# pbs-plus/pbs-plus

Hardware: AMD Instinct MI355X
Metric: GiB/s ingested through CDC+SHA-256 (higher is better)
Workload: dtype u32

## Files before the change

### pbs_plus_amd/csrc/kernels.hip

```cpp
#include "kernel_util.h"
#include "kernels.h"
#include "ring_queue.h"

namespace pbsk {

__device__ __forceinline__ uint32_t rotr(uint32_t x, int n) { return __builtin_rotateright32(x, n); }

__device__ __forceinline__ uint32_t xor3(uint32_t a, uint32_t b, uint32_t c) {
    return __builtin_amdgcn_bitop3_b32(a, b, c, 0x96);
}
__device__ __forceinline__ uint32_t maj3(uint32_t a, uint32_t b, uint32_t c) {
    return __builtin_amdgcn_bitop3_b32(a, b, c, 0xE8);
}
__device__ __forceinline__ uint32_t ch3(uint32_t e, uint32_t f, uint32_t g) { return g ^ (e & (f ^ g)); }

__device__ constexpr uint32_t kSha256K[64] = {
    0x428a2f98, 0x71374491, 0xb5c0fbcf, 0xe9b5dba5, 0x3956c25b, 0x59f111f1, 0x923f82a4, 0xab1c5ed5,
    0xd807aa98, 0x12835b01, 0x243185be, 0x550c7dc3, 0x72be5d74, 0x80deb1fe, 0x9bdc06a7, 0xc19bf174,
    0xe49b69c1, 0xefbe4786, 0x0fc19dc6, 0x240ca1cc, 0x2de92c6f, 0x4a7484aa, 0x5cb0a9dc, 0x76f988da,
    0x983e5152, 0xa831c66d, 0xb00327c8, 0xbf597fc7, 0xc6e00bf3, 0xd5a79147, 0x06ca6351, 0x14292967,
    0x27b70a85, 0x2e1b2138, 0x4d2c6dfc, 0x53380d13, 0x650a7354, 0x766a0abb, 0x81c2c92e, 0x92722c85,
    0xa2bfe8a1, 0xa81a664b, 0xc24b8b70, 0xc76c51a3, 0xd192e819, 0xd6990624, 0xf40e3585, 0x106aa070,
    0x19a4c116, 0x1e376c08, 0x2748774c, 0x34b0bcb5, 0x391c0cb3, 0x4ed8aa4a, 0x5b9cca4f, 0x682e6ff3,
    0x748f82ee, 0x78a5636f, 0x84c87814, 0x8cc70208, 0x90befffa, 0xa4506ceb, 0xbef9a3f7, 0xc67178f2};

__device__ __forceinline__ uint32_t sha256_sched(uint32_t (&W)[16], int i) {
    const uint32_t w15 = W[(i + 1) & 15], w2 = W[(i + 14) & 15];
    const uint32_t s0 = xor3(rotr(w15, 7), rotr(w15, 18), w15 >> 3);
    const uint32_t s1 = xor3(rotr(w2, 17), rotr(w2, 19), w2 >> 10);
    const uint32_t w = W[i & 15] + s0 + W[(i + 9) & 15] + s1;
    W[i & 15] = w;
    return w;
}

#define SHA256_ROUND(a, b, c, d, e, f, g, h, wk)                                   \
    do {                                                                           \
        const uint32_t t1_ = (h) + xor3(rotr(e, 6), rotr(e, 11), rotr(e, 25)) + ch3(e, f, g) + (wk); \
        const uint32_t t2_ = xor3(rotr(a, 2), rotr(a, 13), rotr(a, 22)) + maj3(a, b, c); \
        (d) += t1_;                                                                \
        (h) = t1_ + t2_;                                                           \
    } while (0)

__device__ __forceinline__ void sha256_compress(uint32_t (&H)[8], uint32_t (&W)[16]) {
    uint32_t a = H[0], b = H[1], c = H[2], d = H[3], e = H[4], f = H[5], g = H[6], h = H[7];
#pragma unroll
    for (int i = 0; i < 64; i += 8) {
        uint32_t wk[8];
#pragma unroll
        for (int j = 0; j < 8; ++j) wk[j] = ((i + j < 16) ? W[i + j] : sha256_sched(W, i + j)) + kSha256K[i + j];
        SHA256_ROUND(a, b, c, d, e, f, g, h, wk[0]);
        SHA256_ROUND(h, a, b, c, d, e, f, g, wk[1]);
        SHA256_ROUND(g, h, a, b, c, d, e, f, wk[2]);
        SHA256_ROUND(f, g, h, a, b, c, d, e, wk[3]);
        SHA256_ROUND(e, f, g, h, a, b, c, d, wk[4]);
        SHA256_ROUND(d, e, f, g, h, a, b, c, wk[5]);
        SHA256_ROUND(c, d, e, f, g, h, a, b, wk[6]);
        SHA256_ROUND(b, c, d, e, f, g, h, a, wk[7]);
    }
    H[0] += a; H[1] += b; H[2] += c; H[3] += d; H[4] += e; H[5] += f; H[6] += g; H[7] += h;
}

__device__ __forceinline__ void sha256_iv(uint32_t (&H)[8]) {
    H[0] = 0x6a09e667; H[1] = 0xbb67ae85; H[2] = 0x3c6ef372; H[3] = 0xa54ff53a;
    H[4] = 0x510e527f; H[5] = 0x9b05688c; H[6] = 0x1f83d9ab; H[7] = 0x5be0cd19;
}

__device__ uint32_t kIdleBlock[32];

__device__ __forceinline__ void sha256_request_block(const uint8_t *p, uint32_t (&R)[17], uint32_t &sel) {
    const uint32_t o = (uint32_t)((uintptr_t)p & 3u);
    const gvec4_ptr q = (gvec4_ptr)(p - o);
    const u32x4_a4 v0 = q[0], v1 = q[1], v2 = q[2], v3 = q[3];
    R[0] = v0.x; R[1] = v0.y; R[2] = v0.z; R[3] = v0.w;
    R[4] = v1.x; R[5] = v1.y; R[6] = v1.z; R[7] = v1.w;
    R[8] = v2.x; R[9] = v2.y; R[10] = v2.z; R[11] = v2.w;
    R[12] = v3.x; R[13] = v3.y; R[14] = v3.z; R[15] = v3.w;
    R[16] = ((gword_ptr)(p - o))[o ? 16 : 15];
    sel = ((o) << 24) | ((o + 1) << 16) | ((o + 2) << 8) | (o + 3);
}

__device__ __forceinline__ void sha256_tail_words(const uint8_t *base, uint64_t len, uint64_t off, bool last, uint32_t (&R)[17]) {
    const int64_t rem = (int64_t)len - (int64_t)off;
    const uint32_t valid = rem <= 0 ? 0u : (rem >= 64 ? 64u : (uint32_t)rem);
    uint32_t q[17];
#pragma unroll
    for (int j = 0; j < 17; ++j) q[j] = 0;
    uint32_t o = 0;
    if (valid) {
        const uint8_t *p = base + off;
        o = (uint32_t)((uintptr_t)p & 3u);
        const gword_ptr a = (gword_ptr)(p - o);
        const uint32_t jmax = (o + valid - 1u) >> 2;
#pragma unroll
        for (int j = 0; j < 17; ++j) q[j] = a[min((uint32_t)j, jmax)];
    }
    const uint32_t sh = o * 8u;
#pragma unroll
    for (int j = 0; j < 16; ++j) {
        uint32_t w = sh ? ((q[j] >> sh) | (q[j + 1] << (32u - sh))) : q[j];
        const int32_t k = (int32_t)valid - 4 * j;
        const uint32_t mask = k >= 4 ? 0xffffffffu : (k <= 0 ? 0u : ((1u << (8 * k)) - 1u));
        w &= mask;
        if (rem >= 0 && rem < 64 && k >= 0 && k < 4) w |= 0x80u << (8 * k);
        R[j] = w;
    }
    if (last) {
        const uint64_t bits = len * 8;
        R[14] = __builtin_bswap32((uint32_t)(bits >> 32));
        R[15] = __builtin_bswap32((uint32_t)bits);
    }
    R[16] = 0;
}

struct RecordSource {
    static constexpr bool kRing = false;
    pbsgpu_record *recs;
    const uint4 *qdesc;
    __device__ __forceinline__ void get(uint32_t i, const uint8_t *&ptr, uint64_t &len, uint8_t *&dst) const {
        const uint4 d = qdesc[i];
        ptr = reinterpret_cast<const uint8_t *>(((uint64_t)d.y << 32) | d.x);
        len = d.z;
        dst = recs[d.w].digest;
    }
};
struct SegmentSource {
    static constexpr bool kRing = false;
    const uint8_t *data;
    const pbsgpu_segment *segs;
    uint8_t *digests;
    __device__ __forceinline__ void get(uint32_t i, const uint8_t *&ptr, uint64_t &len, uint8_t *&dst) const {
        ptr = data + segs[i].offset;
        len = segs[i].length;
        dst = digests + (uint64_t)i * 32;
    }
};


struct RingProbe {
    uint32_t n = 0, idle = 0, act = 0;
    unsigned long long c0 = 0, w0 = 0;
};
__device__ __forceinline__ void ring_probe_step(const RingSource &src, RingProbe &pb, const bool busy, const int slot, const int lane,
                                                const uint32_t active = 0) {
    pb.idle |= busy ? 0u : 1u;
    pb.act += active;
    if (++pb.n < kRingProbeSteps) return;
    const unsigned long long c = clock64(), w = wall_clock64();
    if (!pb.idle && pb.w0 != 0ull && lane == 0 && src.probe) {
        atomicAdd(src.probe + slot, (unsigned long long)kRingProbeSteps);
        atomicAdd(src.probe + slot + 1, c - pb.c0);
        atomicAdd(src.probe + slot + 2, w - pb.w0);
        if (slot == 0) atomicAdd(src.probe + 8, (unsigned long long)pb.act);
    }
    pb.n = 0;
    pb.act = 0;
    pb.idle = 0;
    pb.c0 = c;
    pb.w0 = w;
}

template <typename Source>
__global__ __launch_bounds__(64) void k_sha256(Source src, const uint32_t *nitems_p, uint32_t nitems_imm,
                                               uint32_t *queue, const uint32_t *wg_limit, uint32_t whole_chip) {
    if (wg_limit) {
        const uint32_t lim = *wg_limit;
        if (whole_chip ? lim == 0 : blockIdx.x >= lim * 2u) return;
    }
    const int lane = threadIdx.x & 63;
    const uint32_t nitems = nitems_p ? *nitems_p : nitems_imm;

    const uint8_t *base = nullptr;
    uint64_t len = 0;
    uint64_t blk = 0, nblk = 0;
    uint8_t *dst = nullptr;
    bool have = false;
    bool exhausted = false;

    uint32_t R[17];
    uint32_t sel = 0x00010203u;
#pragma unroll
    for (int j = 0; j < 17; ++j) R[j] = 0;

    uint32_t H[8];
    sha256_iv(H);

    auto load_block = [&]() {
        const uint64_t off = blk * 64;
        if (off + 64 <= len) {
            const uint8_t *p = base + off;
            const uint32_t o = (uint32_t)((uintptr_t)p & 3u);
            const gvec4_ptr q = (gvec4_ptr)(p - o);
            const u32x4_a4 v0 = q[0], v1 = q[1], v2 = q[2], v3 = q[3];
            R[0] = v0.x; R[1] = v0.y; R[2] = v0.z; R[3] = v0.w;
            R[4] = v1.x; R[5] = v1.y; R[6] = v1.z; R[7] = v1.w;
            R[8] = v2.x; R[9] = v2.y; R[10] = v2.z; R[11] = v2.w;
            R[12] = v3.x; R[13] = v3.y; R[14] = v3.z; R[15] = v3.w;
            R[16] = o ? ((gword_ptr)(p - o))[16] : 0u;
            sel = ((o) << 24) | ((o + 1) << 16) | ((o + 2) << 8) | (o + 3);
        } else {
            sha256_tail_words(base, len, off, blk + 1 == nblk, R);
            sel = 0x00010203u;
        }
    };

    auto acquire = [&](bool need) {
        const unsigned long long m = __ballot(need);
        if (m == 0) return;
        const uint32_t first = wave_claim(queue, m, (uint32_t)__popcll(m), lane);
        if (need) {
            const uint32_t i = first + wave_rank(m, lane);
            if (i < nitems) {
                src.get(i, base, len, dst);
                blk = 0;
                nblk = (len + 8) / 64 + 1;
                have = true;
            } else {
                exhausted = true;
                have = false;
            }
        }
    };

    acquire(true);
    if (have) load_block();

    while (__any(have)) {
        uint32_t W[16];
#pragma unroll
        for (int j = 0; j < 16; ++j) W[j] = __builtin_amdgcn_perm(R[j + 1], R[j], sel);
        const bool cur = have;
        const bool cur_last = have && (blk + 1 == nblk);
        uint8_t *cur_dst = dst;

        if (have) {
            if (!cur_last) ++blk; else have = false;
        }
        acquire(!have && !exhausted);
        if (have) load_block();

        if (cur) sha256_compress(H, W);

        if (cur_last) {
            uint32_t *o = reinterpret_cast<uint32_t *>(cur_dst);
#pragma unroll
            for (int j = 0; j < 8; ++j) o[j] = __builtin_bswap32(H[j]);
            sha256_iv(H);
        }
    }
}

__global__ __launch_bounds__(512) void k_sha256_lanes(RingSource src) {
    const int lane = threadIdx.x & 63;
    const uint8_t *base = nullptr, *base2 = nullptr;
    uint64_t len = 0, blk = 0, nblk = 0;
    uint32_t len1 = 0, pages = 0xffffffffu, poll_ctr = 0;
    uint8_t *dst = nullptr;
    bool have = false, exhausted = false;
    uint32_t R[17];
    uint32_t sel = 0x00010203u;
#pragma unroll
    for (int j = 0; j < 17; ++j) R[j] = 0;
    uint32_t H[8];
    sha256_iv(H);

    auto load_block = [&]() {
        const uint64_t off = blk * 64;
        const uint8_t *bb = (off < len1) ? base : base2;
        if (off + 64 <= len) {
            sha256_request_block(bb + off, R, sel);
        } else {
            sha256_tail_words(bb, len, off, blk + 1 == nblk, R);
            sel = 0x00010203u;
        }
    };
    auto acquire = [&](bool need) {
        if (__ballot(need) == 0) return;
        if (__ballot(have) != 0 && ((++poll_ctr) & src.poll_mask) != 0u) return;
        uint32_t sh;
        const int32_t avail = ring_queue_avail(&src.ctl->sq, sh);
        const unsigned long long mn = __ballot(need);
        if (avail > 0) {
            const uint32_t cnt = min((uint32_t)__popcll(mn), (uint32_t)avail);
            const uint32_t first = ring_cas_claim(&src.ctl->shead, sh, cnt, mn, lane);
            if (first != 0xffffffffu) {
                const uint32_t rank = wave_rank(mn, lane);
                const bool got = need && rank < cnt;
                uint4 e0, e1;
                ring_desc_load(src.sdesc, (first + rank) & src.smask, got, e0, e1);
                ring_desc_take(src, got, e0, e1, base, base2, len, len1, dst, pages);
                blk = got ? 0ull : blk;
                nblk = got ? ((uint64_t)e0.z + 8u) / 64u + 1u : nblk;
                have = have | got;
            }
        } else if (ring_stop_raised(src) && ring_drained_after_stop(&src.ctl->sq)) {
            exhausted = exhausted | need;
        }
    };

    const bool probe_on = src.probe != nullptr && blockIdx.x == 0 && threadIdx.x < 64;
    uint32_t pn = 0, pidle = 0, pact = 0;
    unsigned long long pw0 = 0;
    acquire(true);
    if (have) load_block();
    for (;;) {
        if (probe_on) {
            const unsigned long long hm = __ballot(have);
            pidle |= hm ? 0u : 1u;
            pact += (uint32_t)__popcll(hm);
            if (++pn >= kRingProbeSteps) {
                const unsigned long long w = wall_clock64();
                if (!pidle && pw0 != 0ull && lane == 0) {
                    atomicAdd(src.probe + 6, (unsigned long long)kRingProbeSteps);
                    atomicAdd(src.probe + 7, w - pw0);
                    atomicAdd(src.probe + 9, (unsigned long long)pact);
                }
                pn = 0; pidle = 0; pact = 0; pw0 = w;
            }
        }
        if (!__any(have)) {
            if (__ballot(!exhausted) == 0ull) break;
            __builtin_amdgcn_s_sleep(48);
            poll_ctr = 0;
            acquire(!exhausted);
            if (have) load_block();
            continue;
        }
        uint32_t W[16];
#pragma unroll
        for (int j = 0; j < 16; ++j) W[j] = __builtin_amdgcn_perm(R[j + 1], R[j], sel);
        const bool cur = have;
        const bool cur_last = have && (blk + 1 == nblk);
        uint8_t *cur_dst = dst;
        if (have) {
            if (!cur_last) ++blk; else have = false;
        }
        if (cur_last) ring_release_pages(src, pages);
        acquire(!have && !exhausted);
        if (have) load_block();
        if (cur) sha256_compress(H, W);
        if (cur_last) {
            PBSK_GLOBAL uint32_t *o = (PBSK_GLOBAL uint32_t *)cur_dst;
#pragma unroll
            for (int j = 0; j < 8; ++j) o[j] = __builtin_bswap32(H[j]);
            ring_cell_publish(o);
            sha256_iv(H);
        }
    }
}

template <typename Source, bool DENSE>
__global__ __launch_bounds__(DENSE ? 512 : 256) void k_sha256_pair(Source src, const uint32_t *nitems_p, uint32_t nitems_imm,
                                                                   uint32_t *queue, const uint32_t *wg_limit) {
    if (wg_limit) {
        const uint32_t lim = *wg_limit;
        if (DENSE ? lim == 0 : blockIdx.x >= lim) return;
    }
    constexpr int NP = DENSE ? 4 : 2;
    __shared__ uint4 wkbuf_[NP][2][16][64];
    __shared__ uint32_t ctrl_[NP][2][64];
    __shared__ uint8_t *dstp_[NP][2][64];
    __shared__ uint32_t alive[NP][2];
    __shared__ uint32_t curw[NP][2];
    const int lane = threadIdx.x & 63;
    const int wave = threadIdx.x >> 6;
    const int pr = (wave & 1) | (wave >= 4 ? 2 : 0);
    const bool producer = (wave >= 2 && wave < 6);
    auto &wkbuf = wkbuf_[pr];
    auto &ctrl = ctrl_[pr];
    auto &dstp = dstp_[pr];
    auto any_alive = [&](const int pb) -> uint32_t {
        uint32_t a = alive[0][pb] | alive[1][pb];
        if constexpr (DENSE) a |= alive[2][pb] | alive[3][pb];
        return a;
    };

    if (producer) {
        const uint32_t nitems = nitems_p ? *nitems_p : nitems_imm;
        const uint8_t *base = nullptr;
        uint64_t len = 0, blk = 0, nblk = 0;
        uint8_t *dst = nullptr;
        bool have = false, exhausted = false;
        [[maybe_unused]] const uint8_t *base2 = nullptr;
        [[maybe_unused]] uint32_t len1 = 0, pages = 0xffffffffu, claim = 0;
        [[maybe_unused]] uint32_t claimed = 0;
        [[maybe_unused]] unsigned long long idle_since = 0;
        [[maybe_unused]] uint32_t hb_seen = 0;
        constexpr int D = 2;
        uint32_t R[D][17];
        uint32_t selv[D], cflag[D];
        uint8_t *dstv[D];
        [[maybe_unused]] uint32_t pagesv[D];
#pragma unroll
        for (int s = 0; s < D; ++s) {
#pragma unroll
            for (int j = 0; j < 17; ++j) R[s][j] = 0;
            selv[s] = 0x00010203u;
            cflag[s] = 0;
            dstv[s] = nullptr;
            pagesv[s] = 0xffffffffu;
        }

        constexpr uint32_t kReserve = 16;
        uint32_t res_next = 0, res_end = 0;
        [[maybe_unused]] uint32_t poll_ctr = 0;
        auto acquire = [&](bool need) {
            if constexpr (Source::kRing) {
                if (__ballot(need) == 0) return;
                if (__ballot(have) != 0 && ((++poll_ctr) & src.poll_mask) != 0u) return;
                const bool long_only = src.long_bytes != 0u && src.xp == 0u && (lane & 15) == 0;
                const bool elig = need && claimed == 0u;
                if (src.long_bytes && __ballot(elig)) {
                    uint32_t lh;
                    int32_t avail = ring_queue_avail(&src.ctl->lq, lh) - (int32_t)src.long_spill;
                    if (avail > 0 && src.xp != 0u && (uint32_t)avail <= src.xp_pairs &&
                        __hip_atomic_load(&src.ctl->xp_busy, __ATOMIC_RELAXED, __HIP_MEMORY_SCOPE_AGENT) < src.xp_pairs)
                        avail = 0;
                    if (avail > 0) {
                        const unsigned long long mn = __ballot(elig);
                        const uint32_t cnt = min((uint32_t)__popcll(mn), (uint32_t)avail);
                        const uint32_t first = ring_cas_claim(&src.ctl->lhead, lh, cnt, mn, lane);
                        if (first != 0xffffffffu) {
                            const uint32_t rank = wave_rank(mn, lane);
                            const bool tk = elig && rank < cnt;
                            uint4 e0, e1;
                            ring_desc_load(src.ldesc, (first + rank) & src.lmask, tk, e0, e1);
                            ring_desc_take(src, tk, e0, e1, base, base2, len, len1, dst, pages);
                            blk = tk ? 0ull : blk;
                            nblk = tk ? ((uint64_t)e0.z + 8u) / 64u + 1u : nblk;
                            have = have | tk;
                            need = need && !tk;
                        }
                    }
                }
                const bool want = need && !claimed && !long_only;
                const unsigned long long mw = __ballot(want);
                if (mw) {
                    uint32_t first = 0;
                    const int leader = __ffsll((long long)mw) - 1;
                    if (lane == leader) {
                        const uint32_t cnt = (uint32_t)__popcll(mw);
                        first = atomicAdd(&src.ctl->head, cnt);
                        if (((first + cnt) ^ first) >> 8)
                            __hip_atomic_store(const_cast<uint32_t *>(src.heartbeat) + 32, first + cnt, __ATOMIC_RELAXED,
                                               __HIP_MEMORY_SCOPE_SYSTEM);
                    }
                    first = __shfl(first, leader, 64);
                    if (want) {
                        claim = first + wave_rank(mw, lane);
                        claimed = 1u;
                    }
                }
                if (__ballot(need) == 0) return;
                const unsigned long long ts = __hip_atomic_load(&src.ctl->tail_stop,
                                                                __ATOMIC_RELAXED, __HIP_MEMORY_SCOPE_AGENT);
                const uint32_t tail = (uint32_t)ts, stop = (uint32_t)(ts >> 32);
                const bool ready = need && claimed != 0u && (int32_t)(tail - claim) > 0;
                if (__ballot(ready)) __atomic_thread_fence(__ATOMIC_ACQUIRE);
                uint4 d0, d1;
                ring_desc_load(src.desc, claim & src.qmask, ready, d0, d1);
                const bool got = ready && d0.z != 0u;
                claimed = ready ? 0u : claimed;
                ring_desc_take(src, got, d0, d1, base, base2, len, len1, dst, pages);
                blk = got ? 0ull : blk;
                nblk = got ? ((uint64_t)d0.z + 8u) / 64u + 1u : nblk;
                have = have | got;
                bool leave = need && !ready && stop != 0u;
                if (src.long_bytes && src.xp == 0u && __ballot(leave) && !ring_drained_after_stop(&src.ctl->lq)) leave = false;
                exhausted = exhausted | leave;
                return;
            }
            const unsigned long long m = __ballot(need);
            if (m == 0) return;
            uint32_t first = 0;
            uint32_t avail = 0;
            if constexpr (DENSE) {
                const uint32_t cnt = (uint32_t)__popcll(m);
                avail = res_end - res_next;
                if (cnt > avail) first = wave_claim(queue, m, cnt - avail + kReserve, lane);
            } else {
                first = wave_claim(queue, m, (uint32_t)__popcll(m), lane);
            }
            if (need) {
                uint32_t i = first + wave_rank(m, lane);
                if constexpr (DENSE) {
                    const uint32_t r = wave_rank(m, lane);
                    i = r < avail ? res_next + r : first + (r - avail);
                }
                if (i < nitems) {
                    if constexpr (!Source::kRing) src.get(i, base, len, dst);
                    blk = 0;
                    nblk = (len + 8) / 64 + 1;
                    have = true;
                } else {
                    exhausted = true;
                    have = false;
                }
            }
            if constexpr (DENSE) {
                const uint32_t cnt = (uint32_t)__popcll(m);
                if (cnt > avail) {
                    res_next = first + (cnt - avail);
                    res_end = res_next + kReserve;
                } else {
                    res_next += cnt;
                }
            }
        };
        auto prep = [&](const int s) {
            acquire(!have && !exhausted);
            uint32_t c = 0;
            const uint8_t *p = reinterpret_cast<const uint8_t *>(kIdleBlock);
            const uint8_t *bb = base;
            uint64_t off = 0;
            bool tail = false, last = false;
            if (have) {
                off = blk * 64;
                if constexpr (Source::kRing) bb = (off < len1) ? base : base2;
                last = blk + 1 == nblk;
                if (off + 64 <= len) p = bb + off;
                else tail = true;
                c = 1u | (last ? 2u : 0u);
                dstv[s] = dst;
                if constexpr (Source::kRing) pagesv[s] = pages;
                if (++blk == nblk) have = false;
            }
            sha256_request_block(p, R[s], selv[s]);
            if (tail) {
                sha256_tail_words(bb, len, off, last, R[s]);
                selv[s] = 0x00010203u;
            }
            cflag[s] = c;
        };

#pragma unroll
        for (int s = 0; s < D; ++s) prep(s);
        bool drained = false;
        [[maybe_unused]] bool wg_busy = false;
        [[maybe_unused]] RingProbe probe;
        [[maybe_unused]] const bool probe_on = blockIdx.x == 0 && wave == 2;
        while (!drained) {
#pragma unroll
            for (int s = 0; s < D; ++s) {
                {
                    constexpr int kBufMask = 1;
                    const int pb = s & kBufMask;
                    uint32_t W[16];
#pragma unroll
                    for (int j = 0; j < 16; ++j) {
                        W[j] = __builtin_amdgcn_perm(R[s][j + 1], R[s][j], selv[s]);
                        asm volatile("" : "+v"(W[j]));
                    }
                    __builtin_amdgcn_sched_barrier(0);
                    const uint32_t c = cflag[s];
                    uint8_t *cur_dst = dstv[s];
                    if constexpr (Source::kRing) {
                        if (c & 2u) ring_release_pages(src, pagesv[s]);
                    }
                    prep(s);
                    const bool any_cur = __any(c & 1u);
                    if (any_cur) {
#pragma unroll
                        for (int q = 0; q < 16; ++q) {
                            uint32_t x[4];
#pragma unroll
                            for (int j = 0; j < 4; ++j) {
                                const int t = 4 * q + j;
                                x[j] = ((t < 16) ? W[t] : sha256_sched(W, t)) + kSha256K[t];
                            }
                            wkbuf[pb][q][lane] = make_uint4(x[0], x[1], x[2], x[3]);
                        }
                    }
                    ctrl[pb][lane] = c;
                    dstp[pb][lane] = cur_dst;
                    bool live = any_cur;
                    if constexpr (Source::kRing) {
                        const bool wave_done = __ballot(!exhausted) == 0ull;
                        live = any_cur || !wave_done;
                        if (!any_cur && !wave_done) {
                            const unsigned long long now = wall_clock64();
                            if (idle_since == 0) idle_since = now;
                            if (blockIdx.x == 0 && wave == 2 && now - idle_since > src.idle_ticks) {
                                uint32_t *hbw = const_cast<uint32_t *>(src.heartbeat);
                                const uint32_t hb = __hip_atomic_load(hbw + kHbBeat, __ATOMIC_RELAXED, __HIP_MEMORY_SCOPE_SYSTEM);
                                if (hb != hb_seen) {
                                    hb_seen = hb;
                                    idle_since = now;
                                } else {
                                    if (lane == 0) __hip_atomic_store(hbw + kHbIntent, 1u, __ATOMIC_RELAXED, __HIP_MEMORY_SCOPE_SYSTEM);
                                    __atomic_thread_fence(__ATOMIC_SEQ_CST);
                                    __threadfence_system();
                                    const uint32_t hb2 = __hip_atomic_load(hbw + kHbBeat, __ATOMIC_RELAXED, __HIP_MEMORY_SCOPE_SYSTEM);
                                    const uint32_t enq = __hip_atomic_load(hbw + kHbRoundsEnq, __ATOMIC_RELAXED, __HIP_MEMORY_SCOPE_SYSTEM);
                                    const uint32_t done = __hip_atomic_load(&src.ctl->rounds_done, __ATOMIC_RELAXED, __HIP_MEMORY_SCOPE_AGENT);
                                    if (hb2 != hb || enq != done) {
                                        if (lane == 0) __hip_atomic_store(hbw + kHbIntent, 0u, __ATOMIC_RELAXED, __HIP_MEMORY_SCOPE_SYSTEM);
                                        hb_seen = hb2;
                                        idle_since = now;
                                    } else if (lane == 0) {
                                        __hip_atomic_store(&src.ctl->stop, 2u, __ATOMIC_RELEASE, __HIP_MEMORY_SCOPE_AGENT);
                                        __hip_atomic_store(hbw + kHbCommitted, 1u, __ATOMIC_RELAXED, __HIP_MEMORY_SCOPE_SYSTEM);
                                    }
                                }
                            }
                            if (!wg_busy) __builtin_amdgcn_s_sleep(48);
                        } else {
                            idle_since = 0;
                        }
                        if (lane == 0) curw[pr][pb] = any_cur ? 1u : 0u;
                        if (probe_on) ring_probe_step(src, probe, any_cur, 0, lane, (uint32_t)__popcll(__ballot(c & 1u)));
                    }
                    if (lane == 0) alive[pr][pb] = live ? 1u : 0u;
                    __syncthreads();
                    drained = drained || __builtin_amdgcn_readfirstlane(any_alive(pb)) == 0u;
                    if constexpr (Source::kRing) {
                        uint32_t w = curw[0][pb] | curw[1][pb];
                        if constexpr (DENSE) w |= curw[2][pb] | curw[3][pb];
                        wg_busy = w != 0u;
                    }
                }
            }
        }
    } else {
        uint32_t H[8];
        sha256_iv(H);
        struct Blk {
            uint32_t al, c;
            uint8_t *d;
            uint4 wk[16];
        };
        auto fetch = [&](Blk &x, const int pb) {
            x.al = any_alive(pb);
            x.c = ctrl[pb][lane];
            x.d = dstp[pb][lane];
#pragma unroll
            for (int q = 0; q < 16; ++q) x.wk[q] = wkbuf[pb][q][lane];
        };
        auto rounds = [&](const Blk &x) {
            if (x.c & 1u) {
                uint32_t a = H[0], b = H[1], cc = H[2], dd = H[3], e = H[4], f = H[5], g = H[6], h = H[7];
#pragma unroll
                for (int q = 0; q < 16; q += 2) {
                    SHA256_ROUND(a, b, cc, dd, e, f, g, h, x.wk[q].x);
                    SHA256_ROUND(h, a, b, cc, dd, e, f, g, x.wk[q].y);
                    SHA256_ROUND(g, h, a, b, cc, dd, e, f, x.wk[q].z);
                    SHA256_ROUND(f, g, h, a, b, cc, dd, e, x.wk[q].w);
                    SHA256_ROUND(e, f, g, h, a, b, cc, dd, x.wk[q + 1].x);
                    SHA256_ROUND(dd, e, f, g, h, a, b, cc, x.wk[q + 1].y);
                    SHA256_ROUND(cc, dd, e, f, g, h, a, b, x.wk[q + 1].z);
                    SHA256_ROUND(b, cc, dd, e, f, g, h, a, x.wk[q + 1].w);
                }
                H[0] += a; H[1] += b; H[2] += cc; H[3] += dd; H[4] += e; H[5] += f; H[6] += g; H[7] += h;
                if (x.c & 2u) {
                    PBSK_GLOBAL uint32_t *o = (PBSK_GLOBAL uint32_t *)x.d;
#pragma unroll
                    for (int j = 0; j < 8; ++j) o[j] = __builtin_bswap32(H[j]);
                    if constexpr (Source::kRing) ring_cell_publish(o);
                    sha256_iv(H);
                }
            }
        };
        Blk A, B;
        __syncthreads();
        fetch(A, 0);
        for (;;) {
            if (!A.al) break;
            __syncthreads();
            fetch(B, 1);
            __builtin_amdgcn_sched_barrier(0);
            rounds(A);
            if (!B.al) break;
            __syncthreads();
            fetch(A, 0);
            __builtin_amdgcn_sched_barrier(0);
            rounds(B);
        }
    }
}

#define XP_R(n, x0, x1, x2, x3, kw)                                                     \
    "v_xad_u32 %[nz], " x3 ", %[role], " kw "\n\t"                                      \
    "v_alignbit_b32 %[r1], " x0 ", " x0 ", %[sh1]\n\t"                                  \
    "v_alignbit_b32 %[r2], " x0 ", " x0 ", %[sh2]\n\t"                                  \
    "v_add_u32_dpp %[p], " x1 ", %[nz] quad_perm:[1,0,3,2] row_mask:0xf bank_mask:0xf\n\t" \
    "v_alignbit_b32 %[r3], " x0 ", " x0 ", %[sh3]\n\t"                                  \
    "v_bitop3_b32 %[sel], " x0 ", " x2 ", %[role] bitop3:0x78\n\t"                      \
    "v_bitop3_b32 %[sg], %[r1], %[r2], %[r3] bitop3:0x96\n\t"                           \
    "v_bitop3_b32 %[f], %[sel], " x1 ", " x2 " bitop3:0xca\n\t"                         \
    "v_add3_u32 " n ", %[sg], %[f], %[p]\n\t"
#define XP_TEMPS                                                                                                   \
    [nz] "=&v"(nz), [r1] "=&v"(r1), [r2] "=&v"(r2), [r3] "=&v"(r3), [p] "=&v"(p), [sel] "=&v"(sel), [sg] "=&v"(sg), \
        [f] "=&v"(f)
struct XpRole {
    uint32_t sh1, sh2, sh3, role;
};
template <bool START>
__device__ __forceinline__ void xp_round4(uint32_t &x0, uint32_t &x1, uint32_t &x2, uint32_t &x3, const uint4 kw, const XpRole &R,
                                          const uint32_t hb1 = 0, const uint32_t hb0 = 0) {
    uint32_t n0, n1, n2, n3, nz, r1, r2, r3, p, sel, sg, f;
    if constexpr (START) {
        asm(XP_R("%[n0]", "%[x0]", "%[x1]", "%[x2]", "%[x3]", "%[k0]")
            "v_bitop3_b32 %[n0], %[role], %[hb1], %[n0] bitop3:0xca\n\t"
            XP_R("%[n1]", "%[n0]", "%[x0]", "%[x1]", "%[x2]", "%[k1]")
            "v_bitop3_b32 %[n1], %[role], %[hb0], %[n1] bitop3:0xca\n\t"
            XP_R("%[n2]", "%[n1]", "%[n0]", "%[x0]", "%[x1]", "%[k2]")
            XP_R("%[n3]", "%[n2]", "%[n1]", "%[n0]", "%[x0]", "%[k3]")
            : [n0] "=&v"(n0), [n1] "=&v"(n1), [n2] "=&v"(n2), [n3] "=&v"(n3), XP_TEMPS
            : [x0] "v"(x0), [x1] "v"(x1), [x2] "v"(x2), [x3] "v"(x3), [k0] "v"(kw.x), [k1] "v"(kw.y), [k2] "v"(kw.z), [k3] "v"(kw.w),
              [sh1] "v"(R.sh1), [sh2] "v"(R.sh2), [sh3] "v"(R.sh3), [role] "v"(R.role), [hb1] "v"(hb1), [hb0] "v"(hb0));
    } else {
        asm(XP_R("%[n0]", "%[x0]", "%[x1]", "%[x2]", "%[x3]", "%[k0]")
            XP_R("%[n1]", "%[n0]", "%[x0]", "%[x1]", "%[x2]", "%[k1]")
            XP_R("%[n2]", "%[n1]", "%[n0]", "%[x0]", "%[x1]", "%[k2]")
            XP_R("%[n3]", "%[n2]", "%[n1]", "%[n0]", "%[x0]", "%[k3]")
            : [n0] "=&v"(n0), [n1] "=&v"(n1), [n2] "=&v"(n2), [n3] "=&v"(n3), XP_TEMPS
            : [x0] "v"(x0), [x1] "v"(x1), [x2] "v"(x2), [x3] "v"(x3), [k0] "v"(kw.x), [k1] "v"(kw.y), [k2] "v"(kw.z), [k3] "v"(kw.w),
              [sh1] "v"(R.sh1), [sh2] "v"(R.sh2), [sh3] "v"(R.sh3), [role] "v"(R.role));
    }
    x0 = n3; x1 = n2; x2 = n1; x3 = n0;
}
__device__ __forceinline__ void xp_round2(uint32_t &x0, uint32_t &x1, uint32_t &x2, uint32_t &x3, const uint32_t kw, const XpRole &R) {
    uint32_t n0, n1, nz, r1, r2, r3, p, sel, sg, f;
    asm(XP_R("%[n0]", "%[x0]", "%[x1]", "%[x2]", "%[x3]", "%[k0]")
        XP_R("%[n1]", "%[n0]", "%[x0]", "%[x1]", "%[x2]", "%[k0]")
        : [n0] "=&v"(n0), [n1] "=&v"(n1), XP_TEMPS
        : [x0] "v"(x0), [x1] "v"(x1), [x2] "v"(x2), [x3] "v"(x3), [k0] "v"(kw), [sh1] "v"(R.sh1), [sh2] "v"(R.sh2), [sh3] "v"(R.sh3),
          [role] "v"(R.role));
    x3 = x1; x2 = x0; x1 = n0; x0 = n1;
}
__device__ __forceinline__ uint32_t xp_sel(uint32_t role, uint32_t a, uint32_t b) { return __builtin_amdgcn_bitop3_b32(role, b, a, 0xCA); }

template <typename Source>
__global__ __launch_bounds__(256) void k_sha256_xpair(Source src, const uint32_t *nitems_p, uint32_t nitems_imm, uint32_t *queue,
                                                      const uint32_t *wg_limit) {
    if (wg_limit && *wg_limit == 0) return;
    __shared__ uint4 wkbuf_[2][2][2][16][64];
    __shared__ uint32_t ctrl_[2][2][2][32];
    __shared__ uint8_t *dstp_[2][2][2][32];
    __shared__ uint32_t alive[2][2];
    __shared__ uint32_t curw[2][2];
    const int lane = threadIdx.x & 63;
    const int wave = threadIdx.x >> 6;
    const int pr = wave & 1;
    const bool producer = wave >= 2;
    const bool roleB = (lane & 1) != 0;
    const int ci = lane >> 1;
    auto &wkbuf = wkbuf_[pr];
    auto &ctrl = ctrl_[pr];
    auto &dstp = dstp_[pr];
    auto any_alive = [&](const int pb) -> uint32_t { return alive[0][pb] | alive[1][pb]; };
    for (int i = threadIdx.x; i < 2 * 2 * 2 * 16 * 32; i += 256) {
        const int row = 2 * (i & 31) + 1, q = (i >> 5) & 15, pl = (i >> 9) & 1, pb = (i >> 10) & 1, pp = (i >> 11) & 1;
        wkbuf_[pp][pb][pl][q][row] = make_uint4(1u, 1u, 1u, 1u);
    }
    __syncthreads();

    if (producer) {
        const uint32_t nitems = nitems_p ? *nitems_p : nitems_imm;
        const uint8_t *base = nullptr;
        uint64_t len = 0, blk = 0, nblk = 0;
        uint8_t *dst = nullptr;
        bool have = false, exhausted = false;
        [[maybe_unused]] const uint8_t *base2 = nullptr;
        [[maybe_unused]] uint32_t len1 = 0, pages = 0xffffffffu;
        [[maybe_unused]] unsigned long long idle_since = 0;
        [[maybe_unused]] uint32_t poll_ctr = 0;
        constexpr int D = 2;
        uint32_t R[D][17];
        uint32_t selv[D], cflag[D];
        uint8_t *dstv[D];
        [[maybe_unused]] uint32_t pagesv[D];
#pragma unroll
        for (int s = 0; s < D; ++s) {
#pragma unroll
            for (int j = 0; j < 17; ++j) R[s][j] = 0;
            selv[s] = 0x00010203u;
            cflag[s] = 0;
            dstv[s] = nullptr;
            pagesv[s] = 0xffffffffu;
        }
        auto acquire = [&](bool need) {
            if (__ballot(need) == 0) return;
            bool got = false;
            if constexpr (Source::kRing) {
                if (__ballot(have) != 0 && ((++poll_ctr) & src.poll_mask) != 0u) return;
                uint32_t lh;
                const int32_t avail = ring_queue_avail(&src.ctl->lq, lh);
                const unsigned long long mn = __ballot(need);
                if (avail > 0) {
                    const uint32_t cnt = min((uint32_t)__popcll(mn), (uint32_t)avail);
                    const uint32_t first = ring_cas_claim(&src.ctl->lhead, lh, cnt, mn, lane);
                    if (first != 0xffffffffu) {
                        const uint32_t rank = wave_rank(mn, lane);
                        got = need && rank < cnt;
                        uint4 e0, e1;
                        ring_desc_load(src.ldesc, (first + rank) & src.lmask, got, e0, e1);
                        ring_desc_take(src, got, e0, e1, base, base2, len, len1, dst, pages);
                        if (lane == __ffsll((long long)mn) - 1) atomicAdd(&src.ctl->xp_busy, cnt);
                    }
                } else if (ring_stop_raised(src) && ring_drained_after_stop(&src.ctl->lq)) {
                    exhausted = exhausted | need;
                }
            } else {
                const unsigned long long m = __ballot(need);
                const uint32_t first = wave_claim(queue, m, (uint32_t)__popcll(m), lane);
                if (need) {
                    const uint32_t i = first + wave_rank(m, lane);
                    if (i < nitems) {
                        src.get(i, base, len, dst);
                        got = true;
                    } else {
                        exhausted = true;
                    }
                }
            }
            const int srcl = lane & ~1;
            const bool pgot = __shfl((int)got, srcl, 64) != 0;
            exhausted = __shfl((int)exhausted, srcl, 64) != 0;
            if (__ballot(pgot)) {
                const uint64_t b1 = (uint64_t)__shfl((unsigned long long)reinterpret_cast<uintptr_t>(base), srcl, 64);
                const uint64_t ln = (uint64_t)__shfl((unsigned long long)len, srcl, 64);
                const uint64_t ds = (uint64_t)__shfl((unsigned long long)reinterpret_cast<uintptr_t>(dst), srcl, 64);
                if (pgot) {
                    base = reinterpret_cast<const uint8_t *>(b1);
                    len = ln;
                    dst = reinterpret_cast<uint8_t *>(ds);
                }
                if constexpr (Source::kRing) {
                    const uint64_t b2 = (uint64_t)__shfl((unsigned long long)reinterpret_cast<uintptr_t>(base2), srcl, 64);
                    const uint32_t l1 = (uint32_t)__shfl((int)len1, srcl, 64);
                    const uint32_t pg = (uint32_t)__shfl((int)pages, srcl, 64);
                    if (pgot) {
                        base2 = reinterpret_cast<const uint8_t *>(b2);
                        len1 = l1;
                        pages = pg;
                    }
                }
                if (pgot) {
                    nblk = (len + 8) / 64 + 1;
                    blk = roleB ? 1ull : 0ull;
                    have = blk < nblk;
                }
            }
        };
        auto prep = [&](const int s) {
            const unsigned long long hm = __ballot(have);
            const bool pair_busy = ((hm >> (lane & ~1)) & 3ull) != 0ull;
            acquire(!roleB && !pair_busy && !exhausted);
            uint32_t c = 0;
            const uint8_t *p = reinterpret_cast<const uint8_t *>(kIdleBlock);
            const uint8_t *bb = base;
            uint64_t off = 0;
            bool tail = false, last = false;
            if (have) {
                off = blk * 64;
                if constexpr (Source::kRing) bb = (off < len1) ? base : base2;
                last = blk + 1 == nblk;
                if (off + 64 <= len) p = bb + off;
                else tail = true;
                c = 1u | (last ? 2u : 0u);
                dstv[s] = dst;
                if constexpr (Source::kRing) pagesv[s] = pages;
                blk += 2;
                if (blk >= nblk) have = false;
            }
            sha256_request_block(p, R[s], selv[s]);
            if (tail) {
                sha256_tail_words(bb, len, off, last, R[s]);
                selv[s] = 0x00010203u;
            }
            cflag[s] = c;
        };
        const int wrow = lane & ~1, wplane = lane & 1;

#pragma unroll
        for (int s = 0; s < D; ++s) prep(s);
        bool drained = false;
        [[maybe_unused]] bool wg_busy = false;
        [[maybe_unused]] RingProbe probe;
        [[maybe_unused]] const bool probe_on = blockIdx.x == 0 && wave == 2;
        while (!drained) {
#pragma unroll
            for (int s = 0; s < D; ++s) {
                {
                    const int pb = s & 1;
                    uint32_t W[16];
#pragma unroll
                    for (int j = 0; j < 16; ++j) {
                        W[j] = __builtin_amdgcn_perm(R[s][j + 1], R[s][j], selv[s]);
                        asm volatile("" : "+v"(W[j]));
                    }
                    __builtin_amdgcn_sched_barrier(0);
                    const uint32_t c = cflag[s];
                    uint8_t *cur_dst = dstv[s];
                    if constexpr (Source::kRing) {
                        {
                            const unsigned long long mdone = __ballot((c & 2u) != 0u);
                            if (mdone && lane == (__ffsll((long long)mdone) - 1)) atomicSub(&src.ctl->xp_busy, (uint32_t)__popcll(mdone));
                        }
                        if (c & 2u) ring_release_pages(src, pagesv[s]);
                    }
                    prep(s);
                    const bool any_cur = __any(c & 1u);
                    if (any_cur) {
#pragma unroll
                        for (int q = 0; q < 16; ++q) {
                            uint32_t x[4];
#pragma unroll
                            for (int j = 0; j < 4; ++j) {
                                const int t = 4 * q + j;
                                x[j] = ((t < 16) ? W[t] : sha256_sched(W, t)) + kSha256K[t];
                            }
                            wkbuf[pb][wplane][q][wrow] = make_uint4(x[0], x[1], x[2], x[3]);
                        }
                    }
                    ctrl[pb][wplane][ci] = c;
                    dstp[pb][wplane][ci] = cur_dst;
                    bool live = any_cur;
                    if constexpr (Source::kRing) {
                        const bool wave_done = __ballot(!exhausted) == 0ull;
                        live = any_cur || !wave_done;
                        if (!any_cur && !wave_done && !wg_busy) __builtin_amdgcn_s_sleep(48);
                        if (lane == 0) curw[pr][pb] = any_cur ? 1u : 0u;
                        if (probe_on) ring_probe_step(src, probe, any_cur, 3, lane);
                    }
                    if (lane == 0) alive[pr][pb] = live ? 1u : 0u;
                    __syncthreads();
                    drained = drained || __builtin_amdgcn_readfirstlane(any_alive(pb)) == 0u;
                    if constexpr (Source::kRing) wg_busy = (curw[0][pb] | curw[1][pb]) != 0u;
                }
            }
        }
    } else {
        const XpRole R{roleB ? 2u : 6u, roleB ? 13u : 11u, roleB ? 22u : 25u, roleB ? 0xffffffffu : 0u};
        const uint32_t role = R.role;
        uint32_t ivr[4];
        ivr[0] = roleB ? 0x6a09e667u : 0x510e527fu;
        ivr[1] = roleB ? 0xbb67ae85u : 0x9b05688cu;
        ivr[2] = roleB ? 0x3c6ef372u : 0x1f83d9abu;
        ivr[3] = roleB ? 0xa54ff53au : 0x5be0cd19u;
        uint32_t HR[4] = {ivr[0], ivr[1], ivr[2], ivr[3]};
        struct Blk {
            uint32_t al, c;
            uint8_t *d;
            uint4 wk[16];
        };
        auto fetch = [&](Blk &x, const int pb, const int plane) {
            x.al = any_alive(pb);
            x.c = ctrl[pb][plane][ci];
            x.d = dstp[pb][plane][ci];
#pragma unroll
            for (int q = 0; q < 16; ++q) x.wk[q] = wkbuf[pb][plane][q][lane];
        };
        auto rounds = [&](const Blk &x) {
            if (x.c & 1u) {
                uint32_t x0 = xp_sel(role, HR[0], HR[2]), x1 = xp_sel(role, HR[1], HR[3]), x2 = HR[2], x3 = HR[3];
                xp_round4<true>(x0, x1, x2, x3, x.wk[0], R, HR[1], HR[0]);
#pragma unroll
                for (int g = 1; g < 16; ++g) xp_round4<false>(x0, x1, x2, x3, x.wk[g], R);
                const uint32_t o63 = x0, o62 = x1, o61 = x2, o60 = x3;
                xp_round2(x0, x1, x2, x3, x.wk[15].w, R);
                HR[0] += xp_sel(role, o63, x0);
                HR[1] += xp_sel(role, o62, x1);
                HR[2] += xp_sel(role, o61, o63);
                HR[3] += xp_sel(role, o60, o62);
                if (x.c & 2u) {
                    PBSK_GLOBAL uint32_t *o = (PBSK_GLOBAL uint32_t *)x.d + (roleB ? 0 : 4);
#pragma unroll
                    for (int j = 0; j < 4; ++j) o[j] = __builtin_bswap32(HR[j]);
                    if constexpr (Source::kRing) ring_cell_publish((PBSK_GLOBAL uint32_t *)x.d);
#pragma unroll
                    for (int j = 0; j < 4; ++j) HR[j] = ivr[j];
                }
            }
        };
        Blk E0, O0, E1, O1;
        __syncthreads();
        fetch(E0, 0, 0);
        for (;;) {
            if (!E0.al) break;
            fetch(O0, 0, 1);
            __builtin_amdgcn_sched_barrier(0);
            rounds(E0);
            __syncthreads();
            fetch(E1, 1, 0);
            __builtin_amdgcn_sched_barrier(0);
            rounds(O0);
            if (!E1.al) break;
            fetch(O1, 1, 1);
            __builtin_amdgcn_sched_barrier(0);
            rounds(E1);
            __syncthreads();
            fetch(E0, 0, 0);
            __builtin_amdgcn_sched_barrier(0);
            rounds(O1);
        }
    }
}

__global__ __launch_bounds__(1024) void k_order(const uint8_t *data, const pbsgpu_segment *segs, const pbsgpu_record *recs,
                                                const uint32_t *nrec_p, uint32_t shift, uint4 *qdesc, uint32_t *wg_limit,
                                                uint32_t max_wgs,
                                                const uint32_t *maxcnt, uint32_t cap, uint32_t slack_pct) {
    if (maxcnt && *maxcnt > cap) {
        if (threadIdx.x == 0) *wg_limit = 0;
        return;
    }
    constexpr int BINS = 1024;
    __shared__ uint32_t hist[BINS];
    __shared__ uint32_t base[BINS];
    __shared__ unsigned long long tot_blocks;
    __shared__ uint32_t longest;
    const uint32_t n = *nrec_p;
    for (int i = threadIdx.x; i < BINS; i += blockDim.x) hist[i] = 0;
    if (threadIdx.x == 0) { tot_blocks = 0; longest = 0; }
    __syncthreads();
    unsigned long long my_blocks = 0;
    uint32_t my_long = 0;
    for (uint32_t i = threadIdx.x; i < n; i += blockDim.x) {
        const uint32_t sz = recs[i].size;
        uint32_t b = sz >> shift;
        if (b >= BINS) b = BINS - 1;
        atomicAdd(&hist[BINS - 1 - b], 1u);
        const uint32_t blocks = (sz + 8) / 64 + 1;
        my_blocks += blocks;
        my_long = max(my_long, blocks);
    }
    atomicAdd(&tot_blocks, my_blocks);
    atomicMax(&longest, my_long);
    __syncthreads();
    if (threadIdx.x == 0) {
        uint32_t run = 0;
        for (int i = 0; i < BINS; ++i) { base[i] = run; run += hist[i]; }
        const unsigned long long lg = longest ? longest : 1;
        unsigned long long lanes = (tot_blocks * (100 + slack_pct) / 100 + lg - 1) / lg;
        uint32_t wgs = (uint32_t)((lanes + 127) / 128);
        const uint32_t need = (n + 127) / 128;
        if (wgs > need) wgs = need;
        if (wgs < 1) wgs = 1;
        if (wgs > max_wgs) wgs = max_wgs;
        *wg_limit = wgs;
    }
    __syncthreads();
    for (uint32_t i = threadIdx.x; i < n; i += blockDim.x) {
        uint32_t b = recs[i].size >> shift;
        if (b >= BINS) b = BINS - 1;
        const uint32_t pos = atomicAdd(&base[BINS - 1 - b], 1u);
        const uint64_t p = (uint64_t)(uintptr_t)(data + segs[recs[i].segment].offset + recs[i].end - recs[i].size);
        qdesc[pos] = make_uint4((uint32_t)p, (uint32_t)(p >> 32), recs[i].size, i);
    }
}

bool sha256_dense_pays(uint64_t total_blocks, uint64_t longest_blocks, int num_cus, uint32_t dense_pct) {
    if (!dense_pct) return false;
    if (longest_blocks < 1) longest_blocks = 1;
    return total_blocks * 100ull > (uint64_t)dense_pct * longest_blocks * 128ull * (uint64_t)num_cus;
}

hipError_t launch_order(const uint8_t *data, const pbsgpu_segment *segs, const pbsgpu_record *recs, const uint32_t *nrec,
                        uint32_t max_chunk, uint4 *qdesc, uint32_t *wg_limit, int num_cus, const uint32_t *maxcnt, uint32_t cap, uint32_t slack_pct,
                        hipStream_t st) {
    uint32_t shift = 0;
    while (((uint64_t)max_chunk >> shift) >= 1024) ++shift;
    hipLaunchKernelGGL(k_order, dim3(1), dim3(1024), 0, st, data, segs, recs, nrec, shift, qdesc, wg_limit, (uint32_t)num_cus,
                       maxcnt, cap, slack_pct);
    return hipGetLastError();
}

constexpr size_t kPairLdsPad = 16u << 10;
constexpr size_t kLaneLdsPad = 36u << 10;

template <typename Source>
static hipError_t launch_pair(unsigned grid, bool dense, hipStream_t st, Source src, uint32_t nitems, uint32_t *queue, int form) {
    if (form == 2) {
        hipLaunchKernelGGL((k_sha256_xpair<Source>), dim3(grid * (dense ? 4u : 2u)), dim3(256), 0, st, src, (const uint32_t *)nullptr,
                           nitems, queue, (const uint32_t *)nullptr);
        return hipGetLastError();
    }
    if (dense) {
        hipLaunchKernelGGL((k_sha256_pair<Source, true>), dim3(grid), dim3(512), 0, st, src, (const uint32_t *)nullptr,
                           nitems, queue, (const uint32_t *)nullptr);
    } else {
        const size_t pad = kPairLdsPad;
        hipError_t e = allow_lds(&k_sha256_pair<Source, false>, pad);
        if (e != hipSuccess) return e;
        hipLaunchKernelGGL((k_sha256_pair<Source, false>), dim3(grid), dim3(256), pad, st, src,
                           (const uint32_t *)nullptr, nitems, queue, (const uint32_t *)nullptr);
    }
    return hipGetLastError();
}

hipError_t launch_sha256_records(pbsgpu_record *recs, const uint32_t *nrec, uint32_t *queue, const uint4 *qdesc,
                                 const uint32_t *wg_limit, int num_cus, bool dense, int form, hipStream_t st) {
    RecordSource src{recs, qdesc};
    if (form == 2) {
        hipLaunchKernelGGL((k_sha256_xpair<RecordSource>), dim3((unsigned)num_cus), dim3(256), 0, st, src, nrec, 0u, queue,
                           wg_limit);
    } else if (form == 0) {
        if (dense) {
            hipLaunchKernelGGL((k_sha256_pair<RecordSource, true>), dim3((unsigned)num_cus), dim3(512), 0, st, src, nrec,
                               0u, queue, wg_limit);
        } else {
            hipError_t e = allow_lds(&k_sha256_pair<RecordSource, false>, kPairLdsPad);
            if (e != hipSuccess) return e;
            hipLaunchKernelGGL((k_sha256_pair<RecordSource, false>), dim3((unsigned)num_cus), dim3(256), kPairLdsPad, st, src,
                               nrec, 0u, queue, wg_limit);
        }
    } else {
        hipError_t e = allow_lds(&k_sha256<RecordSource>, kLaneLdsPad);
        if (e != hipSuccess) return e;
        hipLaunchKernelGGL((k_sha256<RecordSource>), dim3((unsigned)num_cus * 4u), dim3(64), kLaneLdsPad, st, src, nrec, 0u,
                           queue, wg_limit, 0u);
    }
    return hipGetLastError();
}

hipError_t launch_sha256_segments(const uint8_t *data, const pbsgpu_segment *segs, uint32_t nseg, uint8_t *digests,
                                  uint32_t *queue, int num_cus, bool dense, int form, hipStream_t st) {
    if (nseg == 0) return hipSuccess;
    SegmentSource src{data, segs, digests};
    if (form != 1) {
        unsigned g2 = (unsigned)num_cus;
        const unsigned need2 = (nseg + (dense ? 255u : 127u)) / (dense ? 256u : 128u);
        if (g2 > need2) g2 = need2;
        return launch_pair(g2, dense, st, src, nseg, queue, form);
    }
    hipError_t e = allow_lds(&k_sha256<SegmentSource>, kLaneLdsPad);
    if (e != hipSuccess) return e;
    const size_t pad = dense ? kLaneLdsPad / 2 : kLaneLdsPad;
    unsigned grid = (unsigned)num_cus * (dense ? 8u : 4u);
    const unsigned need = (nseg + 63) / 64;
    if (grid > need) grid = need;
    hipLaunchKernelGGL((k_sha256<SegmentSource>), dim3(grid), dim3(64), pad, st, src, (const uint32_t *)nullptr,
                       nseg, queue, (const uint32_t *)nullptr, 0u);
    return hipGetLastError();
}

hipError_t launch_ring_service_xp(const RingSource &q, unsigned workgroups, hipStream_t st) {
    hipFuncAttributes fa{};
    hipError_t e = hipFuncGetAttributes(&fa, reinterpret_cast<const void *>(&k_sha256_xpair<RingSource>));
    if (e != hipSuccess) return e;
    size_t pad = (160u << 10) > fa.sharedSizeBytes ? (160u << 10) - fa.sharedSizeBytes : 0;
    pad &= ~(size_t)255;
    e = allow_lds(&k_sha256_xpair<RingSource>, pad);
    if (e != hipSuccess) return e;
    hipLaunchKernelGGL((k_sha256_xpair<RingSource>), dim3(workgroups), dim3(256), pad, st, q, (const uint32_t *)nullptr, 0u,
                       (uint32_t *)nullptr, (const uint32_t *)nullptr);
    return hipGetLastError();
}

hipError_t launch_ring_service_lanes(const RingSource &q, unsigned workgroups, hipStream_t st, bool dense) {
    const size_t pad = (size_t)(160u << 10) & ~(size_t)255;
    hipError_t e = allow_lds(&k_sha256_lanes, pad);
    if (e != hipSuccess) return e;
    hipLaunchKernelGGL(k_sha256_lanes, dim3(workgroups), dim3(dense ? 512 : 256), pad, st, q);
    return hipGetLastError();
}

template <bool DENSE>
static hipError_t launch_ring_service_form(const RingSource &q, unsigned workgroups, hipStream_t st) {
    hipFuncAttributes fa{};
    hipError_t e = hipFuncGetAttributes(&fa, reinterpret_cast<const void *>(&k_sha256_pair<RingSource, DENSE>));
    if (e != hipSuccess) return e;
    size_t pad = (160u << 10) > fa.sharedSizeBytes ? (160u << 10) - fa.sharedSizeBytes : 0;
    pad &= ~(size_t)255;
    e = allow_lds(&k_sha256_pair<RingSource, DENSE>, pad);
    if (e != hipSuccess) return e;
    hipLaunchKernelGGL((k_sha256_pair<RingSource, DENSE>), dim3(workgroups), dim3(DENSE ? 512 : 256), pad, st, q,
                       (const uint32_t *)nullptr, 0u, (uint32_t *)nullptr, (const uint32_t *)nullptr);
    return hipGetLastError();
}
hipError_t launch_ring_service(const RingSource &q, unsigned workgroups, hipStream_t st, bool dense) {
    return dense ? launch_ring_service_form<true>(q, workgroups, st) : launch_ring_service_form<false>(q, workgroups, st);
}

}
```

Baseline: 709.9.

## Pack SHA handshake into one LDS record and make consumer rounds branch-free

Replaces the separate control-word and destination-pointer LDS arrays with one 16-byte record per lane that also carries a drained flag. Consumers now load it with a single vector read and end their loop from that flag instead of reading the shared alive array. The SHA round body now runs unconditionally and only the state update is predicated. Digest write-out sits behind a wave-wide any() test so the common path has no divergent branches. Producers run one extra iteration to publish the drained flag, and idle lanes now compute rounds they throw away.

```diff
diff --git a/pbs_plus_amd/csrc/kernels.hip b/pbs_plus_amd/csrc/kernels.hip
--- a/pbs_plus_amd/csrc/kernels.hip
+++ b/pbs_plus_amd/csrc/kernels.hip
@@ -729,13 +729,22 @@
 }
 __device__ __forceinline__ uint32_t xp_sel(uint32_t role, uint32_t a, uint32_t b) { return __builtin_amdgcn_bitop3_b32(role, b, a, 0xCA); }
 
+constexpr uint32_t kHsValid = 1u, kHsLast = 2u, kHsDrained = 4u;
+typedef uint32_t hs_rec __attribute__((ext_vector_type(4)));
+__device__ __forceinline__ hs_rec hs_record(const uint32_t c, const bool drained, const uint8_t *dst) {
+    const uint64_t d = (uint64_t)reinterpret_cast<uintptr_t>(dst);
+    return hs_rec{(uint32_t)d, (uint32_t)(d >> 32), c | (drained ? kHsDrained : 0u), 0u};
+}
+__device__ __forceinline__ PBSK_GLOBAL uint32_t *hs_dst(const hs_rec &r) {
+    return (PBSK_GLOBAL uint32_t *)(((uint64_t)r.y << 32) | r.x);
+}
+
 template <typename Source>
 __global__ __launch_bounds__(256) void k_sha256_xpair(Source src, const uint32_t *nitems_p, uint32_t nitems_imm, uint32_t *queue,
                                                       const uint32_t *wg_limit) {
     if (wg_limit && *wg_limit == 0) return;
     __shared__ uint4 wkbuf_[2][2][2][16][64];
-    __shared__ uint32_t ctrl_[2][2][2][32];
-    __shared__ uint8_t *dstp_[2][2][2][32];
+    __shared__ hs_rec hs_[2][2][2][32];
     __shared__ uint32_t alive[2][2];
     __shared__ uint32_t curw[2][2];
     const int lane = threadIdx.x & 63;
@@ -745,8 +754,7 @@
     const bool roleB = (lane & 1) != 0;
     const int ci = lane >> 1;
     auto &wkbuf = wkbuf_[pr];
-    auto &ctrl = ctrl_[pr];
-    auto &dstp = dstp_[pr];
+    auto &hs = hs_[pr];
     auto any_alive = [&](const int pb) -> uint32_t { return alive[0][pb] | alive[1][pb]; };
     for (int i = threadIdx.x; i < 2 * 2 * 2 * 16 * 32; i += 256) {
         const int row = 2 * (i & 31) + 1, q = (i >> 5) & 15, pl = (i >> 9) & 1, pb = (i >> 10) & 1, pp = (i >> 11) & 1;
@@ -874,15 +882,16 @@
 
 #pragma unroll
         for (int s = 0; s < D; ++s) prep(s);
-        bool drained = false;
+        bool drained = false, told = false;
         [[maybe_unused]] bool wg_busy = false;
         [[maybe_unused]] RingProbe probe;
         [[maybe_unused]] const bool probe_on = blockIdx.x == 0 && wave == 2;
-        while (!drained) {
+        while (!told) {
 #pragma unroll
             for (int s = 0; s < D; ++s) {
                 {
                     const int pb = s & 1;
+                    if (s == 0) told = drained;
                     uint32_t W[16];
 #pragma unroll
                     for (int j = 0; j < 16; ++j) {
@@ -913,8 +922,7 @@
                             wkbuf[pb][wplane][q][wrow] = make_uint4(x[0], x[1], x[2], x[3]);
                         }
                     }
-                    ctrl[pb][wplane][ci] = c;
-                    dstp[pb][wplane][ci] = cur_dst;
+                    hs[pb][wplane][ci] = hs_record(c, drained, cur_dst);
                     bool live = any_cur;
                     if constexpr (Source::kRing) {
                         const bool wave_done = __ballot(!exhausted) == 0ull;
@@ -940,59 +948,74 @@
         ivr[3] = roleB ? 0xa54ff53au : 0x5be0cd19u;
         uint32_t HR[4] = {ivr[0], ivr[1], ivr[2], ivr[3]};
         struct Blk {
-            uint32_t al, c;
-            uint8_t *d;
+            hs_rec r;
             uint4 wk[16];
         };
         auto fetch = [&](Blk &x, const int pb, const int plane) {
-            x.al = any_alive(pb);
-            x.c = ctrl[pb][plane][ci];
-            x.d = dstp[pb][plane][ci];
 #pragma unroll
             for (int q = 0; q < 16; ++q) x.wk[q] = wkbuf[pb][plane][q][lane];
+            x.r = hs[pb][plane][ci];
         };
         auto rounds = [&](const Blk &x) {
-            if (x.c & 1u) {
-                uint32_t x0 = xp_sel(role, HR[0], HR[2]), x1 = xp_sel(role, HR[1], HR[3]), x2 = HR[2], x3 = HR[3];
-                xp_round4<true>(x0, x1, x2, x3, x.wk[0], R, HR[1], HR[0]);
-#pragma unroll
-                for (int g = 1; g < 16; ++g) xp_round4<false>(x0, x1, x2, x3, x.wk[g], R);
-                const uint32_t o63 = x0, o62 = x1, o61 = x2, o60 = x3;
-                xp_round2(x0, x1, x2, x3, x.wk[15].w, R);
+            uint32_t x0 = xp_sel(role, HR[0], HR[2]), x1 = xp_sel(role, HR[1], HR[3]), x2 = HR[2], x3 = HR[3];
+            xp_round4<true>(x0, x1, x2, x3, x.wk[0], R, HR[1], HR[0]);
+#pragma unroll
+            for (int g = 1; g < 16; ++g) xp_round4<false>(x0, x1, x2, x3, x.wk[g], R);
+            uint32_t o63 = x0, o62 = x1, o61 = x2, o60 = x3;
+            xp_round2(x0, x1, x2, x3, x.wk[15].w, R);
+            asm volatile("" : "+v"(x0), "+v"(x1), "+v"(o60), "+v"(o61), "+v"(o62), "+v"(o63));
+            if (x.r.z != 0u) {
                 HR[0] += xp_sel(role, o63, x0);
                 HR[1] += xp_sel(role, o62, x1);
                 HR[2] += xp_sel(role, o61, o63);
                 HR[3] += xp_sel(role, o60, o62);
-                if (x.c & 2u) {
-                    PBSK_GLOBAL uint32_t *o = (PBSK_GLOBAL uint32_t *)x.d + (roleB ? 0 : 4);
-#pragma unroll
-                    for (int j = 0; j < 4; ++j) o[j] = __builtin_bswap32(HR[j]);
-                    if constexpr (Source::kRing) ring_cell_publish((PBSK_GLOBAL uint32_t *)x.d);
-#pragma unroll
-                    for (int j = 0; j < 4; ++j) HR[j] = ivr[j];
-                }
+            }
+        };
+        auto digest = [&](const Blk &x) {
+            if (x.r.z & kHsLast) {
+                PBSK_GLOBAL uint32_t *o = hs_dst(x.r) + (roleB ? 0 : 4);
+#pragma unroll
+                for (int j = 0; j < 4; ++j) o[j] = __builtin_bswap32(HR[j]);
+                if constexpr (Source::kRing) ring_cell_publish(hs_dst(x.r));
+#pragma unroll
+                for (int j = 0; j < 4; ++j) HR[j] = ivr[j];
+            }
+        };
+        auto ends = [&](const Blk &x) {
+            if (__any(x.r.z > kHsValid)) {
+                asm volatile("");
+                digest(x);
             }
         };
         Blk E0, O0, E1, O1;
         __syncthreads();
         fetch(E0, 0, 0);
         for (;;) {
-            if (!E0.al) break;
             fetch(O0, 0, 1);
             __builtin_amdgcn_sched_barrier(0);
             rounds(E0);
+            asm volatile("" : "+v"(O0.r));
+            ends(E0);
             __syncthreads();
             fetch(E1, 1, 0);
             __builtin_amdgcn_sched_barrier(0);
             rounds(O0);
-            if (!E1.al) break;
+            asm volatile("" : "+v"(E1.r));
+            ends(O0);
             fetch(O1, 1, 1);
             __builtin_amdgcn_sched_barrier(0);
             rounds(E1);
+            asm volatile("" : "+v"(O1.r));
+            ends(E1);
             __syncthreads();
             fetch(E0, 0, 0);
             __builtin_amdgcn_sched_barrier(0);
             rounds(O1);
+            asm volatile("" : "+v"(E0.r));
+            if (__any((O1.r.z | E0.r.z) > kHsValid)) {
+                digest(O1);
+                if (__any(E0.r.z & kHsDrained)) break;
+            }
         }
     }
 }
```

New measurement: 709.9, median of 2. No clear change (-0.0%).
